# MMintLab/gelslim_depth

Hardware: AMD Instinct MI355X
Metric: train frames/sec (320x427) at batch 32 (higher is better)
Workload: dtype f32

## Files before the change

### gelslim_depth_amd/csrc/gsd_conv3x3_w2d.hip

```cpp
#include "gsd_conv3x3_host.h"

#include <cstdio>
#include <cstdlib>
#include <type_traits>

__device__ const float gsd_pad_w2d[2] = {0.f, __builtin_nanf("")};

typedef float f32x4v __attribute__((ext_vector_type(4), aligned(4)));
typedef float f32x2v __attribute__((ext_vector_type(2)));

struct W2DParams {
  SrcD src0, src1;
  DstD dst0, dst1;
  const float* wt;
  float* partials;
  const float* bw_raw;
  const float* bw_scale;
  const float* bw_shift;
  const float* bw_mean;
  const float* bw_invstd;
  int Cin, Cout, Mpad, nchunks, mblocks;
  int N, H, W;
  int TH, TW, TWq, tiles_y, tiles_x, WR, WC, WCp, PS, NPV;
  int NP, NI;
  int mgrp, pgrp, ptiles;
  int nslab;
  float* slabs;
};

namespace {
constexpr int W2D_BM = 64;
constexpr int W2D_WTILE = 96 * W2D_BM;
constexpr int NWP = 2;
}

template <class GetY>
__device__ __forceinline__ void w2d_epilogue(const W2DParams& P, const float* sBw, const int n, const int h0, const int w0, const int tr2,
                                             const int tq, const int vmask, const int m0, const int mh, const int ph, const int j,
                                             const int l16, const int pt, GetY get_y) {
  constexpr int BM = 64;
  int off0_0 = 0, off0_1 = 0, off1_0 = 0, off1_1 = 0, sm0_0 = 0, sm0_1 = 0, sm1_0 = 0, sm1_1 = 0;
#pragma unroll
  for (int a = 0; a < 2; ++a) {
    const int h = h0 + 2 * tr2 + a, w = w0 + 4 * tq;
    const int vm = (vmask >> (4 * a)) & 15;
    int hd = h - P.dst0.oh, wd = w - P.dst0.ow;
    if ((unsigned)hd < (unsigned)P.dst0.H) {
      (a == 0 ? off0_0 : off0_1) = hd * P.dst0.ws + wd;
#pragma unroll
      for (int i = 0; i < 4; ++i)
        if ((vm >> i & 1) && (unsigned)(wd + i) < (unsigned)P.dst0.W) (a == 0 ? sm0_0 : sm0_1) |= 1 << i;
    }
    hd = h - P.dst1.oh;
    wd = w - P.dst1.ow;
    if ((unsigned)hd < (unsigned)P.dst1.H) {
      (a == 0 ? off1_0 : off1_1) = hd * P.dst1.ws + wd;
#pragma unroll
      for (int i = 0; i < 4; ++i)
        if ((vm >> i & 1) && (unsigned)(wd + i) < (unsigned)P.dst1.W) (a == 0 ? sm1_0 : sm1_1) |= 1 << i;
    }
  }
  auto OFF0 = [&](int a) { return a == 0 ? off0_0 : off0_1; };
  auto OFF1 = [&](int a) { return a == 0 ? off1_0 : off1_1; };
  auto SM0 = [&](int a) { return a == 0 ? sm0_0 : sm0_1; };
  auto SM1 = [&](int a) { return a == 0 ? sm1_0 : sm1_1; };
  const long long lane0 = (long long)(j * 4) * P.dst0.cs, lane1 = (long long)(j * 4) * P.dst1.cs;
  float* const d0 = P.dst0.p + (long long)n * P.dst0.ns;
  float* const d1 = P.dst1.p + (long long)n * P.dst1.ns;
  float* const prow = P.partials != nullptr ? P.partials + (size_t)(pt * NWP + ph) * (2 * P.Mpad) : nullptr;

  if (P.bw_raw == nullptr) {
#pragma unroll
    for (int m = 0; m < 2; ++m) {
#pragma unroll
      for (int reg = 0; reg < 4; ++reg) {
        const int cu = m0 + mh * 32 + m * 16 + reg, co = cu + j * 4;
        const bool first = co < P.dst0.C;
        const int cd = first ? co : co - P.dst0.C;
        const bool co_ok = co < P.Cout && (first || cd < P.dst1.C);
        float* const plane = first ? d0 + (long long)cu * P.dst0.cs + lane0 : d1 + (long long)(cu - P.dst0.C) * P.dst1.cs + lane1;
        float y[2][4];
        get_y(m, reg, y);
        float s1 = 0.f, s2 = 0.f;
#pragma unroll
        for (int a = 0; a < 2; ++a) {
          const int sm = co_ok ? (first ? SM0(a) : SM1(a)) : 0;
          float* const px = plane + (first ? OFF0(a) : OFF1(a));
#pragma unroll
          for (int i = 0; i < 4; ++i) {
            if (sm >> i & 1) {
              s1 += y[a][i];
              s2 = fmaf(y[a][i], y[a][i], s2);
            }
          }
          if (sm == 15) {
            *reinterpret_cast<f32x4v*>(px) = f32x4{y[a][0], y[a][1], y[a][2], y[a][3]};
          } else {
#pragma unroll
            for (int i = 0; i < 4; ++i)
              if (sm >> i & 1) px[i] = y[a][i];
          }
        }
        if (prow != nullptr) {
          s1 = reduce16_to_lane15(s1);
          s2 = reduce16_to_lane15(s2);
          if (l16 == 15 && co < P.Mpad) {
            prow[co] = s1;
            prow[P.Mpad + co] = s2;
          }
        }
      }
    }
  } else {
#pragma unroll
    for (int m = 0; m < 2; ++m) {
#pragma unroll
      for (int reg = 0; reg < 4; ++reg) {
        const int cu = m0 + mh * 32 + m * 16 + reg, co = cu + j * 4;
        const long long cplane = (long long)n * P.dst0.ns + (co < P.Cout ? (long long)cu * P.dst0.cs + lane0 : 0);
        float xr[2][4];
#pragma unroll
        for (int a = 0; a < 2; ++a) {
          const float* const rp = P.bw_raw + cplane + OFF0(a);
          if (SM0(a) == 15) {
            const f32x4 t = *reinterpret_cast<const f32x4v*>(rp);
            xr[a][0] = t[0], xr[a][1] = t[1], xr[a][2] = t[2], xr[a][3] = t[3];
          } else {
#pragma unroll
            for (int i = 0; i < 4; ++i) xr[a][i] = (SM0(a) >> i & 1) ? rp[i] : 0.f;
          }
        }
        const int cl = mh * 32 + m * 16 + j * 4 + reg;
        const float bsc = sBw[cl], bsh = sBw[BM + cl], bmu = sBw[2 * BM + cl], bis = sBw[3 * BM + cl];
        float y[2][4];
        get_y(m, reg, y);
        float s1 = 0.f, s2 = 0.f;
#pragma unroll
        for (int a = 0; a < 2; ++a) {
          const int sm = co < P.Cout ? SM0(a) : 0;
          float* const px = d0 + ((long long)cu * P.dst0.cs + lane0) + OFF0(a);
#pragma unroll
          for (int i = 0; i < 4; ++i) {
            const float x = xr[a][i];
            const float dz = ((sm >> i & 1) && fmaf(x, bsc, bsh) > 0.f) ? y[a][i] : 0.f;
            y[a][i] = dz;
            s1 += dz;
            s2 = fmaf(dz, (x - bmu) * bis, s2);
          }
          if (sm == 15) {
            *reinterpret_cast<f32x4v*>(px) = f32x4{y[a][0], y[a][1], y[a][2], y[a][3]};
          } else {
#pragma unroll
            for (int i = 0; i < 4; ++i)
              if (sm >> i & 1) px[i] = y[a][i];
          }
        }
        if (prow != nullptr) {
          s1 = reduce16_to_lane15(s1);
          s2 = reduce16_to_lane15(s2);
          if (l16 == 15 && co < P.Mpad) {
            prow[co] = s1;
            prow[P.Mpad + co] = s2;
          }
        }
      }
    }
  }
}

template <bool PLAIN, int HM = 0, bool SPLIT = false>
__global__ __launch_bounds__(128 * NWP, 2) void conv3x3_w2d_kernel(const W2DParams P) {
  constexpr bool X4 = HM == 1, U4 = HM == 2, PC = HM != 0;
  constexpr int W2D_NONE = -2147483647 - 1, W2D_PAD = -2147483647;
  static_assert(!X4 || PLAIN, "aligned 16-byte halo pieces: a plain, row-pitched source");
  constexpr int BM = W2D_BM, WTILE = W2D_WTILE, NT = 128 * NWP, NW = 2 * NWP;
  extern __shared__ __attribute__((aligned(16))) float smem[];
  const int PS = P.PS;
  const int BUF = WTILE + 4 * PS;

  const int tid = threadIdx.x, lane = tid & 63;
  const int wave8 = __builtin_amdgcn_readfirstlane(tid >> 6);
  const int ph = wave8 % NWP, fh = wave8 / NWP;
  const int j = lane >> 4, l16 = lane & 15;

  const int lid = xcd_swizzle(blockIdx.x, gridDim.x);
  int mbb = lid % P.mblocks;
  const int slab = SPLIT ? (lid / P.mblocks) % P.nslab : 0;
  int pt = SPLIT ? lid / P.mblocks / P.nslab : lid / P.mblocks;
  if (!SPLIT && P.mgrp < P.mblocks) {
    const int gsz = P.pgrp * P.mblocks;
    const int g = lid / gsz;
    int r = lid - g * gsz;
    const int p0 = g * P.pgrp;
    const int pn = min(P.pgrp, P.ptiles - p0);
    const int per = pn * P.mgrp;
    const int mg = r / per;
    r -= mg * per;
    const int gn = min(P.mgrp, P.mblocks - mg * P.mgrp);
    const int pl = r / gn;
    pt = p0 + pl;
    mbb = mg * P.mgrp + (r - pl * gn);
  }
  const int c_lo = SPLIT ? (int)((long)slab * P.nchunks / P.nslab) : 0;
  const int c_hi = SPLIT ? (int)((long)(slab + 1) * P.nchunks / P.nslab) : P.nchunks;
  const int m0 = mbb * BM;
  const int tpi = P.tiles_y * P.tiles_x;
  const int n = pt / tpi;
  const int rt = pt - n * tpi;
  const int ty = rt / P.tiles_x;
  const int h0 = ty * P.TH, w0 = (rt - ty * P.tiles_x) * P.TW;

  const int q = ph * 16 + l16;
  const bool q_ok = q < (P.TH >> 1) * P.TWq && q < 16 * NWP;
  const int tr2 = q_ok ? q / P.TWq : 0;
  const int tq = q_ok ? q - tr2 * P.TWq : 0;
  const int baddr = WTILE + j * PS + (2 * tr2) * P.WCp + 4 * tq + (PC ? 4 : 0);
  int vmask = 0;
  if (q_ok) {
#pragma unroll
    for (int a = 0; a < 2; ++a)
      if (h0 + 2 * tr2 + a < P.H) {
#pragma unroll
        for (int i = 0; i < 4; ++i)
          if (w0 + 4 * tq + i < P.W) vmask |= 1 << (4 * a + i);
      }
  }

  bool p_on[2];
  int pmask = 0;
  auto seg_offsets = [&](const int seg, int (&xo)[2], const bool mark) __attribute__((always_inline)) {
    const SrcD& S = seg ? P.src1 : P.src0;
#pragma unroll
    for (int pp = 0; pp < 2; ++pp) {
      xo[pp] = W2D_NONE;
      if constexpr (PC) {
        const int u = wave8 + NW * pp;
        p_on[pp] = u < 4 * P.NI;
        const int piece = (u % P.NI) * 64 + lane;
        const int rr = piece / P.NP, pc = piece - rr * P.NP;
        if (rr < P.WR) {
          const int gh = h0 - 1 + rr, gw = w0 - 4 + 4 * pc;
          if constexpr (X4) {
            xo[pp] = ((unsigned)gh < (unsigned)S.H && gw >= 0 && gw + 4 <= S.ws) ? gh * S.ws + gw : W2D_PAD;
          } else {
            const int hs = gh - S.oh, c0 = gw - S.ow;
            xo[pp] = W2D_PAD;
            if (S.C > 0 && (unsigned)hs < (unsigned)S.H && c0 + 3 >= 0 && c0 < S.W) {
              xo[pp] = hs * S.ws + c0;
#pragma unroll
              for (int e = 0; e < 4; ++e)
                if (mark && (c0 + e < 0 || c0 + e >= S.W)) pmask |= 1 << (8 * seg + 4 * pp + e);
            }
          }
        }
        continue;
      }
      p_on[pp] = wave8 + NW * pp < P.NPV;
      const int pos = (wave8 + NW * pp) * 64 + lane;
      const int rr = pos / P.WCp, cc = pos - rr * P.WCp;
      if (rr < P.WR && cc < P.WC) {
        const int gh = h0 - 1 + rr, gw = w0 - 1 + cc;
        const int hs = gh - S.oh, ws = gw - S.ow;
        xo[pp] = ((unsigned)hs < (unsigned)S.H && (unsigned)ws < (unsigned)S.W) ? hs * S.ws + ws : W2D_PAD;
      }
    }
  };
  int xo0[2], xo1[2];
  seg_offsets(0, xo0, true);
  seg_offsets(1, xo1, true);
  const int f_sw = P.src1.C > 0 ? P.src0.C / 4 : -1;
  const bool start1 = SPLIT && f_sw >= 0 && c_lo >= f_sw;
  {
    const float pad0 = (start1 ? P.src1.relu : P.src0.relu) ? __builtin_nanf("") : 0.f;
#pragma unroll
    for (int pp = 0; pp < 2; ++pp)
      if (p_on[pp] && (start1 ? xo1[pp] : xo0[pp]) == W2D_PAD) {
#pragma unroll
        for (int b = 0; b < 2; ++b) {
          if constexpr (PC) {
            const int u = wave8 + NW * pp;
#pragma unroll
            for (int e = 0; e < 4; ++e) smem[b * BUF + WTILE + (u / P.NI) * PS + 1 + (u % P.NI) * 256 + lane * 4 + e] = pad0;
          } else {
#pragma unroll
            for (int ch = 0; ch < 4; ++ch) smem[b * BUF + WTILE + ch * PS + (wave8 + NW * pp) * 64 + lane] = pad0;
          }
        }
      }
  }
  long long d_cs = start1 ? P.src1.cs : P.src0.cs;
  const float* d_base = (start1 ? P.src1.p + (long long)n * P.src1.ns : P.src0.p + (long long)n * P.src0.ns) +
                        (long long)(c_lo - (start1 ? f_sw : 0)) * 4 * d_cs;
  long long f_xl[2];
#pragma unroll
  for (int pp = 0; pp < 2; ++pp) f_xl[pp] = start1 ? xo1[pp] : xo0[pp];
  auto begin_fill = [&](int chunk, int buf) {
    if (f_sw < 0 || start1 || (chunk != f_sw && chunk != f_sw + 1)) return;
    if (chunk == f_sw) {
      d_base = P.src1.p + (long long)n * P.src1.ns;
      d_cs = P.src1.cs;
      int xs[2];
      seg_offsets(1, xs, false);
#pragma unroll
      for (int pp = 0; pp < 2; ++pp) f_xl[pp] = xs[pp];
    }
    const float pad1 = P.src1.relu ? __builtin_nanf("") : 0.f;
#pragma unroll
    for (int pp = 0; pp < 2; ++pp)
      if (p_on[pp] && f_xl[pp] == W2D_PAD) {
        if constexpr (PC) {
          const int u = wave8 + NW * pp;
#pragma unroll
          for (int e = 0; e < 4; ++e) smem[buf * BUF + WTILE + (u / P.NI) * PS + 1 + (u % P.NI) * 256 + lane * 4 + e] = pad1;
        } else {
#pragma unroll
          for (int ch = 0; ch < 4; ++ch) smem[buf * BUF + WTILE + ch * PS + (wave8 + NW * pp) * 64 + lane] = pad1;
        }
      }
  };
  auto halo_slot = [&](int ch, float* Xb) {
#pragma unroll
    for (int pp = 0; pp < 2; ++pp)
      if (p_on[pp] && f_xl[pp] > W2D_PAD) __builtin_amdgcn_global_load_lds(d_base + f_xl[pp], Xb + ch * PS + (wave8 + NW * pp) * 64, 4, 0, 0);
    d_base += d_cs;
  };
  auto halo_unit = [&](int pp, float* Xb) {
    const int u = wave8 + NW * pp;
    if (p_on[pp] && f_xl[pp] > W2D_PAD)
      __builtin_amdgcn_global_load_lds(d_base + (u / P.NI) * d_cs + f_xl[pp], Xb + (u / P.NI) * PS + 1 + (u % P.NI) * 256, 16, 0, 0);
    if (pp == 1) d_base += 4 * d_cs;
  };
  constexpr int WPW = 24 / NW;
  const float* const wsrc0 = P.wt + (size_t)mbb * P.nchunks * WTILE + wave8 * (WPW * 256) + lane * 4;
  auto weight_fill = [&](int chunk, float* Wn) {
    const float* wg = wsrc0 + (size_t)chunk * WTILE;
    float* wl = Wn + wave8 * (WPW * 256);
    __builtin_amdgcn_global_load_lds(wg, wl, 16, 0, 0);
    __builtin_amdgcn_global_load_lds(wg, wl, 16, 1024, 0);
    __builtin_amdgcn_global_load_lds(wg, wl, 16, 2048, 0);
    if constexpr (WPW == 6) {
      __builtin_amdgcn_global_load_lds(wg, wl, 16, 3072, 0);
      __builtin_amdgcn_global_load_lds(wg + 1024, wl + 1024, 16, 0, 0);
      __builtin_amdgcn_global_load_lds(wg + 1024, wl + 1024, 16, 1024, 0);
    }
  };

  const int Kpad = P.nchunks * 4;
  float* sAff = smem + 2 * BUF;
  for (int c = tid; c < Kpad; c += NT) {
    const bool first = c < P.src0.C;
    const SrcD& S = first ? P.src0 : P.src1;
    const int cc = first ? c : c - P.src0.C;
    float sc = 1.f, sh = 0.f;
    if (c < P.Cin && cc < S.C && S.scale != nullptr) {
      sc = S.scale[cc];
      sh = S.shift[cc];
    }
    sAff[c] = sc;
    sAff[Kpad + c] = sh;
  }
  float* sBw = sAff + 2 * Kpad;
  if (P.bw_raw != nullptr) {
    for (int c = tid; c < BM; c += NT) {
      const int co = m0 + c < P.Cout ? m0 + c : 0;
      sBw[c] = P.bw_scale[co];
      sBw[BM + c] = P.bw_shift[co];
      sBw[2 * BM + c] = P.bw_mean[co];
      sBw[3 * BM + c] = P.bw_invstd[co];
    }
  }
  const float lo0 = P.src0.relu ? 0.f : -__builtin_inff(), lo1 = P.src1.relu ? 0.f : -__builtin_inff();

  const int rowA = baddr + (fh ? 2 : 0) * P.WCp, rowB = baddr + (fh ? 1 : 2) * P.WCp, rowC = baddr + (fh ? 3 : 1) * P.WCp;
  const f32x2v sg2 = {fh ? -1.f : 1.f, fh ? -1.f : 1.f};

  f32x4 acc[4][12];
#pragma unroll
  for (int m = 0; m < 4; ++m)
#pragma unroll
    for (int f = 0; f < 12; ++f) acc[m][f] = f32x4{0.f, 0.f, 0.f, 0.f};

  const int a_keep = (j * 12 + fh * 6) * 128 + l16 * 4 + fh * 64, a_give = a_keep + (fh ? -64 : 64);
  begin_fill(c_lo, 0);
  weight_fill(c_lo, smem);
  if constexpr (PC) {
    halo_unit(0, smem + WTILE);
    halo_unit(1, smem + WTILE);
  } else {
#pragma unroll
    for (int ch = 0; ch < 4; ++ch) halo_slot(ch, smem + WTILE);
  }

  auto run_chunk = [&](const int chunk, auto cur_c) {
    constexpr int cur = decltype(cur_c)::value;
    if constexpr (U4) {
      __builtin_amdgcn_s_waitcnt(0x0F70);
      const bool seg1 = f_sw >= 0 && chunk >= f_sw;
      const int pm = seg1 ? pmask >> 8 : pmask & 0xff;
      if (pm != 0) {
        const float padv = (seg1 ? P.src1.relu : P.src0.relu) ? __builtin_nanf("") : 0.f;
#pragma unroll
        for (int pp = 0; pp < 2; ++pp) {
          const int u = wave8 + NW * pp;
          float* pq = smem + cur * BUF + WTILE + (u / P.NI) * PS + 1 + (u % P.NI) * 256 + lane * 4;
#pragma unroll
          for (int e = 0; e < 4; ++e)
            if (pm >> (4 * pp + e) & 1) pq[e] = padv;
        }
      }
      __syncthreads();
    } else {
      gsd_dma_barrier();
    }
    const int kc = chunk * 4 + j;
    float sc = 1.f, sh = 0.f, lo = 0.f;
    if constexpr (!PLAIN) {
      sc = sAff[kc], sh = sAff[Kpad + kc];
      lo = kc < P.src0.C ? lo0 : (kc < P.Cin ? lo1 : -__builtin_inff());
    }
    const bool more = chunk + 1 < c_hi;
    int ioff = cur * BUF;
    __asm__ volatile("" : "+s"(ioff));
    const float* Wc = smem + ioff;
    auto load_row = [&](const int addr, float (&r)[6]) {
      const f32x4 ra = *reinterpret_cast<const f32x4*>(&Wc[addr]);
      const f32x2v rb = *reinterpret_cast<const f32x2v*>(&Wc[addr + 4]);
      r[0] = ra[0], r[1] = ra[1], r[2] = ra[2], r[3] = ra[3], r[4] = rb[0], r[5] = rb[1];
    };
    float dA[6], dB[6], dC[6];
    load_row(rowA, dA);
    load_row(rowB, dB);
    load_row(rowC, dC);
    f32x4 av[2];
    av[0] = *reinterpret_cast<const f32x4*>(&Wc[a_keep]);
    auto affine = [&](float (&r)[6]) {
      if constexpr (!PLAIN) {
        const f32x2v sc2 = {sc, sc}, sh2 = {sh, sh};
#pragma unroll
        for (int c = 0; c < 6; c += 2) {
          const f32x2v y = __builtin_elementwise_fma(f32x2v{r[c], r[c + 1]}, sc2, sh2);
          r[c] = fmaxf(y[0], lo);
          r[c + 1] = fmaxf(y[1], lo);
        }
      }
    };
    const f32x2v m41 = {-4.f, -1.f}, p1m1 = {1.f, -1.f}, p2m2 = {2.f, -2.f}, m5 = {-5.f, -5.f}, p4 = {4.f, 4.f};
    auto rt_a = [&](const f32x2v (&tp)[3], f32x2v& ac, f32x2v& be) {
      ac = __builtin_elementwise_fma(f32x2v{tp[1][0], tp[1][0]}, m41, f32x2v{tp[2][0], tp[2][0]});
      be = __builtin_elementwise_fma(f32x2v{tp[0][1], tp[0][1]}, m41, f32x2v{tp[1][1], tp[1][1]});
    };
    auto rt_b = [&](const f32x2v& ac, const f32x2v& be, float (&v)[6]) {
      const f32x2v v12 = __builtin_elementwise_fma(f32x2v{be[0], be[0]}, p1m1, f32x2v{ac[0], ac[0]});
      const f32x2v v34 = __builtin_elementwise_fma(f32x2v{be[1], be[1]}, p2m2, f32x2v{ac[1], ac[1]});
      v[1] = v12[0], v[2] = v12[1], v[3] = v34[0], v[4] = v34[1];
    };
    auto rt_c = [&](const f32x2v (&tp)[3], float (&v)[6]) {
      const f32x2v v05 = __builtin_elementwise_fma(tp[0], p4, __builtin_elementwise_fma(tp[1], m5, tp[2]));
      v[0] = v05[0], v[5] = v05[1];
    };
    affine(dA);
    affine(dB);
    f32x2v tA[3], tB[3], acB, beB;
#pragma unroll
    for (int k = 0; k < 3; ++k) tA[k] = f32x2v{dA[2 * k], dA[2 * k + 1]} - f32x2v{dB[2 * k], dB[2 * k + 1]};
    auto col_b = [&]() {
#pragma unroll
      for (int k = 0; k < 3; ++k)
        tB[k] = __builtin_elementwise_fma(f32x2v{dC[2 * k], dC[2 * k + 1]}, sg2, f32x2v{dB[2 * k], dB[2 * k + 1]});
    };
    if constexpr (!PLAIN) {
      affine(dC);
      col_b();
    }
    float v[2][6];
    {
      f32x2v ac, be;
      rt_a(tA, ac, be);
      rt_b(ac, be, v[0]);
      rt_c(tA, v[0]);
    }
    __builtin_amdgcn_sched_barrier(0);
#pragma unroll
    for (int g = 0; g < 12; ++g) {
      const int r = g / 6, fe = (g >> 1) * 2 - 6 * r, mt = 2 * (g & 1);
      if (g + 1 < 12) av[(g + 1) & 1] = *reinterpret_cast<const f32x4*>(&Wc[((g + 1) & 1 ? a_give : a_keep) + ((g + 1) >> 1) * 128]);
      const f32x4& ap = av[g & 1];
      acc[mt][6 * r + fe] = mfma16(ap[0], v[r][fe], acc[mt][6 * r + fe]);
      acc[mt + 1][6 * r + fe] = mfma16(ap[1], v[r][fe], acc[mt + 1][6 * r + fe]);
      acc[mt][6 * r + fe + 1] = mfma16(ap[2], v[r][fe + 1], acc[mt][6 * r + fe + 1]);
      acc[mt + 1][6 * r + fe + 1] = mfma16(ap[3], v[r][fe + 1], acc[mt + 1][6 * r + fe + 1]);
      const int piece = PLAIN ? g + 1 : g + 2;
      if (piece == 1) col_b();
      if (piece == 2) rt_a(tB, acB, beB);
      if (piece == 3) rt_b(acB, beB, v[1]);
      if (piece == 4) rt_c(tB, v[1]);
      if (more && g < 3) {
        float* Wn = smem + (cur ^ 1) * BUF;
        if (g == 0) {
          begin_fill(chunk + 1, cur ^ 1);
          weight_fill(chunk + 1, Wn);
        } else {
          if constexpr (PC) {
            halo_unit(g - 1, Wn + WTILE);
          } else {
            halo_slot(2 * g - 2, Wn + WTILE);
            halo_slot(2 * g - 1, Wn + WTILE);
          }
        }
      }
      if (g < 6) {
#pragma unroll
        for (int i = 0; i < 4; ++i) {
          __builtin_amdgcn_sched_group_barrier(0x008, 1, 0);
          __builtin_amdgcn_sched_group_barrier(0x002, 1, 0);
        }
      }
      __builtin_amdgcn_sched_barrier(0);
    }
  };
  for (int chunk = c_lo; chunk < c_hi; chunk += 2) {
    run_chunk(chunk, std::integral_constant<int, 0>{});
    if (chunk + 1 < c_hi) run_chunk(chunk + 1, std::integral_constant<int, 1>{});
  }

  {
    float* const xs = smem + (wave8 * 12) * 256 + lane * 4;
    const float* const xr = smem + ((ph + NWP * (1 - fh)) * 12) * 256 + lane * 4;
#pragma unroll
    for (int r = 0; r < 2; ++r) {
      __syncthreads();
#pragma unroll
      for (int f = 0; f < 12; ++f) *reinterpret_cast<f32x4*>(xs + f * 256) = acc[2 + r][f];
      __syncthreads();
#pragma unroll
      for (int f = 0; f < 12; ++f) acc[2 + r][f] = *reinterpret_cast<const f32x4*>(xr + f * 256);
    }
  }

  auto out_transform = [&](auto hi_c, int m, int reg, float (&y)[2][4]) __attribute__((always_inline)) {
    constexpr bool HI = decltype(hi_c)::value;
    const int lo = HI ? 2 + m : m, hi = HI ? m : 2 + m;
    const int r0 = reg & ~1;
#pragma unroll
    for (int a = 0; a < 2; ++a) {
      f32x2v R[6];
#pragma unroll
      for (int fc = 0; fc < 6; ++fc) {
        const f32x2v M0 = {acc[lo][fc][r0], acc[lo][fc][r0 + 1]}, M1 = {acc[lo][6 + fc][r0], acc[lo][6 + fc][r0 + 1]};
        const f32x2v M2 = {acc[hi][fc][r0], acc[hi][fc][r0 + 1]}, M3 = {acc[hi][6 + fc][r0], acc[hi][6 + fc][r0 + 1]};
        R[fc] = a == 0 ? M0 + M1 + M2 : M1 - M2 - M3;
      }
      const f32x2v p12 = R[1] + R[2], m12 = R[1] - R[2], p34 = R[3] + R[4], m34 = R[3] - R[4];
      const f32x2v c2 = {2.f, 2.f}, c4 = {4.f, 4.f}, c8 = {8.f, 8.f};
      const f32x2v y0 = R[0] + p12 + p34, y1 = __builtin_elementwise_fma(c2, m34, m12), y2 = __builtin_elementwise_fma(c4, p34, p12);
      const f32x2v y3 = __builtin_elementwise_fma(c8, m34, m12) + R[5];
      y[a][0] = y0[reg & 1], y[a][1] = y1[reg & 1], y[a][2] = y2[reg & 1], y[a][3] = y3[reg & 1];
    }
  };

  auto finish = [&](auto hi_c) __attribute__((always_inline)) {
    auto get_y = [&](int m, int reg, float (&y)[2][4]) __attribute__((always_inline)) { out_transform(hi_c, m, reg, y); };
    if constexpr (SPLIT) {
      float* const sl = P.slabs + ((size_t)((size_t)pt * P.nslab + slab) * P.mblocks + mbb) * (size_t)(BM * 128 * NWP);
#pragma unroll
      for (int m = 0; m < 2; ++m)
#pragma unroll
        for (int reg = 0; reg < 4; ++reg) {
          float y[2][4];
          get_y(m, reg, y);
          float* const o = sl + ((size_t)(fh * 32 + m * 16 + j * 4 + reg) * (16 * NWP) + q) * 8;
          *reinterpret_cast<f32x4*>(o) = f32x4{y[0][0], y[0][1], y[0][2], y[0][3]};
          *reinterpret_cast<f32x4*>(o + 4) = f32x4{y[1][0], y[1][1], y[1][2], y[1][3]};
        }
    } else {
      w2d_epilogue(P, sBw, n, h0, w0, tr2, tq, vmask, m0, fh, ph, j, l16, pt, get_y);
    }
  };
  if (fh == 0)
    finish(std::false_type{});
  else
    finish(std::true_type{});
}

__global__ __launch_bounds__(128 * NWP) void w2d_slab_reduce_kernel(const W2DParams P) {
  constexpr int BM = W2D_BM;
  __shared__ float sBw[4 * BM];
  const int tid = threadIdx.x, lane = tid & 63;
  const int wave8 = __builtin_amdgcn_readfirstlane(tid >> 6);
  const int ph = wave8 % NWP, mh = wave8 / NWP;
  const int j = lane >> 4, l16 = lane & 15;
  const int lid = xcd_swizzle(blockIdx.x, gridDim.x);
  const int mbb = lid % P.mblocks;
  const int pt = lid / P.mblocks;
  const int m0 = mbb * BM;
  const int tpi = P.tiles_y * P.tiles_x;
  const int n = pt / tpi;
  const int rt = pt - n * tpi;
  const int ty = rt / P.tiles_x;
  const int h0 = ty * P.TH, w0 = (rt - ty * P.tiles_x) * P.TW;
  const int q = ph * 16 + l16;
  const bool q_ok = q < (P.TH >> 1) * P.TWq && q < 16 * NWP;
  const int tr2 = q_ok ? q / P.TWq : 0;
  const int tq = q_ok ? q - tr2 * P.TWq : 0;
  int vmask = 0;
  if (q_ok) {
#pragma unroll
    for (int a = 0; a < 2; ++a)
      if (h0 + 2 * tr2 + a < P.H) {
#pragma unroll
        for (int i = 0; i < 4; ++i)
          if (w0 + 4 * tq + i < P.W) vmask |= 1 << (4 * a + i);
      }
  }
  if (P.bw_raw != nullptr) {
    for (int c = tid; c < BM; c += 128 * NWP) {
      const int co = m0 + c < P.Cout ? m0 + c : 0;
      sBw[c] = P.bw_scale[co];
      sBw[BM + c] = P.bw_shift[co];
      sBw[2 * BM + c] = P.bw_mean[co];
      sBw[3 * BM + c] = P.bw_invstd[co];
    }
    __syncthreads();
  }
  const size_t tile_elems = (size_t)(BM * 128 * NWP);
  const float* const s0 = P.slabs + ((size_t)pt * P.nslab * P.mblocks + mbb) * tile_elems;
  auto get_y = [&](int m, int reg, float (&y)[2][4]) __attribute__((always_inline)) {
    const float* o = s0 + ((size_t)(mh * 32 + m * 16 + j * 4 + reg) * (16 * NWP) + q) * 8;
    f32x4 a = *reinterpret_cast<const f32x4*>(o), b = *reinterpret_cast<const f32x4*>(o + 4);
    for (int s = 1; s < P.nslab; ++s) {
      o += (size_t)P.mblocks * tile_elems;
      a += *reinterpret_cast<const f32x4*>(o);
      b += *reinterpret_cast<const f32x4*>(o + 4);
    }
    y[0][0] = a[0], y[0][1] = a[1], y[0][2] = a[2], y[0][3] = a[3];
    y[1][0] = b[0], y[1][1] = b[1], y[1][2] = b[2], y[1][3] = b[3];
  };
  w2d_epilogue(P, sBw, n, h0, w0, tr2, tq, vmask, m0, mh, ph, j, l16, pt, get_y);
}

namespace {

struct W2DPlan {
  int TH, TW, TWq, tiles_y, tiles_x, mblocks, WR, WC, WCp, PS;
};

bool plan_w2d(int N, int H, int W, int M, W2DPlan* best) {
  long best_cost = -1;
  const int force_tw = gsd_env_int("GSD_W2D_TW", 0);
  const int maxpos = 256 * NWP;
  static const int tws[4] = {32, 64, 16, 8};
  for (int k = 0; k < 4; ++k) {
    const int tw = tws[k];
    if (force_tw && tw != force_tw) continue;
    const int twq = tw / 4;
    int th = 2 * (16 * NWP / twq);
    const int wcp0 = round_up(tw + 2, 4);
    if ((th + 2) * wcp0 > maxpos) continue;
    const int ty = ceil_div(H, th);
    th = round_up(ceil_div(H, ty), 2);
    const long blocks = (long)ty * ceil_div(W, tw) * N;
    const long cost = (blocks * 8 + (tw == 32 ? 0 : tw == 64 ? 1 : tw == 16 ? 2 : 3)) * (tw == 8 ? 100 + gsd_env_int("GSD_W2D_TW8_PCT", 8) : 100);
    if (best_cost < 0 || cost < best_cost) {
      best_cost = cost;
      best->TH = th; best->TW = tw; best->TWq = twq;
      best->tiles_y = ty; best->tiles_x = ceil_div(W, tw);
      best->WR = th + 2; best->WC = tw + 2;
    }
  }
  best->mblocks = ceil_div(M, W2D_BM);
  if (best_cost < 0) return false;
  static std::atomic<uint64_t> memo[16];
  const int th = best->TH, tw = best->TW, key = (th << 16) | (tw << 4);
  std::atomic<uint64_t>& mm = memo[(th * 7 + tw) & 15];
  {
    const uint64_t v = mm.load(std::memory_order_acquire);
    if (v != 0 && (int)(v >> 40) == key) {
      best->WCp = (int)(v >> 20) & 0xFFFFF;
      best->PS = (int)v & 0xFFFFF;
      return true;
    }
  }
  const int wcp0 = round_up(tw + 2, 4);
  int bc = -1;
  for (int c = wcp0; c <= wcp0 + 12 && (th + 2) * c <= maxpos; c += 4)
    for (int ps = round_up((th + 2) * c, 4) + 4; ps < round_up((th + 2) * c, 4) + 4 + 36; ps += 4) {
      const int cyc = conv3_halo_read_cycles(NWP, 2, best->TWq, c, ps, 0);
      if (bc < 0 || cyc < bc) {
        bc = cyc;
        best->WCp = c;
        best->PS = ps;
      }
    }
  if (key < (1 << 24) && best->WCp < (1 << 20) && best->PS < (1 << 20))
    mm.store(((uint64_t)key << 40) | ((uint64_t)best->WCp << 20) | (uint64_t)best->PS, std::memory_order_release);
  return true;
}

int w2d_x4_plane_stride(int TWq, int WCp, int WR) {
  static std::atomic<uint64_t> memo[8];
  const int key = (TWq << 20) | (WCp << 8) | WR;
  std::atomic<uint64_t>& mm = memo[(TWq + WR) & 7];
  {
    const uint64_t v = mm.load(std::memory_order_acquire);
    if (v != 0 && (int)(v >> 32) == key) return (int)(v & 0xFFFFFFFFu);
  }
  int best = -1, ps_best = WR * WCp + 4;
  for (int ps = WR * WCp + 4; ps < WR * WCp + 4 + 68; ps += 4) {
    const int c = conv3_halo_read_cycles(NWP, 2, TWq, WCp, ps, 0);
    if (best < 0 || c < best) {
      best = c;
      ps_best = ps;
    }
  }
  mm.store(((uint64_t)(unsigned)key << 32) | (uint64_t)(unsigned)ps_best, std::memory_order_release);
  return ps_best;
}

template <bool PLAIN, int HM = 0, bool SPLIT = false>
int launch_w2d(const W2DParams& P, int grid, size_t lds, hipStream_t st) {
  if (int e = gsd_launch<conv3x3_w2d_kernel<PLAIN, HM, SPLIT>>("gsd_conv3x3_w2d", dim3(grid), dim3(128 * NWP), lds, st, P)) return e;
  if constexpr (SPLIT) {
    hipLaunchKernelGGL(w2d_slab_reduce_kernel, dim3(grid / P.nslab), dim3(128 * NWP), 0, st, P);
    GSD_LAUNCH_CHECK("gsd_conv3x3_w2d (slab sums)");
  }
  return GSD_OK;
}

constexpr Conv3SlabModel w2d_slabs = {2.07, 5.0, 0.66, "GSD_W2D_SPLIT"};

}

extern "C" int gsd_conv3x3_w2d_supported(int Cin, int C0) {
  return (Cin > 0 && Cin % 4 == 0 && C0 > 0 && C0 <= Cin && C0 % 4 == 0) ? 1 : 0;
}

extern "C" int gsd_conv3x3_w2d_partial_rows(int N, int H, int W, int Cout) {
  if (N <= 0 || H <= 0 || W <= 0 || Cout <= 0) return 0;
  W2DPlan p;
  if (!plan_w2d(N, H, W, Cout, &p)) return 0;
  return N * p.tiles_y * p.tiles_x * NWP;
}

extern "C" int64_t gsd_conv3x3_w2d_mfma_count(int N, int H, int W, int Cin, int Cout) {
  W2DPlan p;
  if (N <= 0 || H <= 0 || W <= 0 || Cin <= 0 || Cout <= 0 || !plan_w2d(N, H, W, Cout, &p)) return 0;
  return (int64_t)N * p.tiles_y * p.tiles_x * p.mblocks * ceil_div(Cin, 4) * (2 * NWP * 48);
}

extern "C" double gsd_conv3x3_w2d_estimate_us(int N, int H, int W, int Cin, int Cout) {
  W2DPlan p;
  if (N <= 0 || H <= 0 || W <= 0 || Cin <= 0 || Cout <= 0 || !plan_w2d(N, H, W, Cout, &p)) return 0.0;
  const long blocks = (long)N * p.tiles_y * p.tiles_x * p.mblocks;
  return w2d_slabs.time_us(blocks, ceil_div(Cin, 4), 1, false);
}

extern "C" double gsd_conv3x3_w2d_estimate_slabs_us(int N, int H, int W, int Cin, int Cout) {
  W2DPlan p;
  if (N <= 0 || H <= 0 || W <= 0 || Cin <= 0 || Cout <= 0 || !plan_w2d(N, H, W, Cout, &p)) return 0.0;
  const long blocks = (long)N * p.tiles_y * p.tiles_x * p.mblocks;
  return w2d_slabs.time_us(blocks, ceil_div(Cin, 4), w2d_slabs.pick(blocks, ceil_div(Cin, 4), false), false);
}

extern "C" int64_t gsd_conv3x3_w2d_workspace(int N, int H, int W, int Cin, int Cout) {
  W2DPlan p;
  if (N <= 0 || H <= 0 || W <= 0 || Cin <= 0 || Cout <= 0 || Cin % 4 != 0 || !plan_w2d(N, H, W, Cout, &p)) return 0;
  const long blocks = (long)N * p.tiles_y * p.tiles_x * p.mblocks;
  const int S = std::max(w2d_slabs.pick(blocks, Cin / 4, false), w2d_slabs.pick(blocks, Cin / 4, true));
  return S > 1 ? (int64_t)blocks * S * (W2D_BM * 256) : 0;
}

extern "C" int gsd_conv3x3_prefers_w2d(int N, int H, int W, int Cin, int Cout, int train) {
  if (N <= 0 || H <= 0 || W <= 0 || Cin < 16 || Cin % 4 != 0 || Cout <= 0) return 0;
  const int forced = gsd_env_int("GSD_CONV_W2D", -1);
  if (forced == 0 || forced == 1) return forced;
  if (!train) return 1;
  const double a = gsd_conv3x3_w2d_estimate_slabs_us(N, H, W, Cin, Cout), b = gsd_conv3x3_w43_estimate_us(N, H, W, Cin, Cout, 1);
  return a > 0.0 && b > 0.0 && a < b ? 1 : 0;
}

static int w2d_impl(const gsd_src* src, int nsrc, const float* wt, int Cin, int Cout, const gsd_dst* dst, int ndst, float* partials,
                    const Conv3Bw& bw, int N, int H, int W, void* stream, float* ws = nullptr, int64_t ws_elems = 0) {
  if (int e = conv3_check_operands("gsd_conv3x3_w2d", true, true, src, nsrc, wt, Cin, Cout, dst, ndst, N, H, W)) return e;
  GSD_REQUIRE(gsd_conv3x3_w2d_supported(Cin, src[0].C), GSD_ERR_UNSUPPORTED,
              "gsd_conv3x3_w2d: Cin=%d and the first segment's %d channels must be multiples of 4 (use gsd_conv3x3_w43)", Cin, src[0].C);

  W2DPlan pl;
  GSD_REQUIRE(plan_w2d(N, H, W, Cout, &pl), GSD_ERR_UNSUPPORTED, "gsd_conv3x3_w2d: no tile shape");
  W2DParams P;
  conv3_fill_common(P, src, nsrc, wt, Cin, Cout, dst, ndst, partials, bw, N, H, W);
  P.mblocks = pl.mblocks;
  P.TH = pl.TH; P.TW = pl.TW; P.TWq = pl.TWq; P.tiles_y = pl.tiles_y; P.tiles_x = pl.tiles_x;
  P.WR = pl.WR; P.WC = pl.WC; P.WCp = pl.WCp; P.PS = pl.PS;
  P.NPV = ceil_div(P.WR * P.WCp, 64);
  GSD_REQUIRE(P.NPV <= 4 * NWP, GSD_ERR_UNSUPPORTED, "gsd_conv3x3_w2d: halo window too large");
  {
    int g = (gsd_env_int("GSD_W2D_L2KB", 3072) << 10) / (P.nchunks * W2D_WTILE * 4);
    const int forced = gsd_env_int("GSD_W2D_MGROUP", -1);
    if (forced == 0) g = P.mblocks;
    if (forced > 0) g = forced;
    P.mgrp = std::min(std::max(g, 1), P.mblocks);
    P.pgrp = std::max(gsd_env_int("GSD_W2D_PGROUP", 64 / P.mgrp), 1);
    P.ptiles = N * pl.tiles_y * pl.tiles_x;
  }
  const long base = (long)N * pl.tiles_y * pl.tiles_x * P.mblocks;
  int S = ws != nullptr ? w2d_slabs.pick(base, P.nchunks, bw.raw != nullptr) : 1;
  while (S > 1 && (int64_t)base * S * (W2D_BM * 256) > ws_elems) --S;
  if (S > 1 && P.nchunks / S < 2) S = 1;
  P.nslab = S;
  P.slabs = S > 1 ? ws : nullptr;
  if (S > 1) GSD_REQUIRE(((uintptr_t)ws & 15) == 0, GSD_ERR_BAD_ARG, "gsd_conv3x3_w2d: the K-slab workspace must be 16-byte aligned");
  const long grid = base * S;
  GSD_REQUIRE(grid < 2147483647L, GSD_ERR_UNSUPPORTED, "gsd_conv3x3_w2d: grid too large");
  bool plain = true;
  for (int i = 0; i < nsrc; ++i) plain = plain && src[i].scale == nullptr && src[i].relu == 0;
  P.NP = pl.TW / 4 + 2;
  P.NI = ceil_div(P.WR * P.NP, 64);
  const bool x4 = plain && nsrc == 1 && 4 * P.NI <= 8 && gsd_env_int("GSD_W2D_X4", 1) != 0 &&
                  ((uintptr_t)src[0].ptr & 15) == 0 && src[0].w_stride % 4 == 0 && src[0].c_stride % 4 == 0 && src[0].n_stride % 4 == 0 &&
                  src[0].off_h == 0 && src[0].off_w == 0 && src[0].w_stride >= round_up(src[0].W, 4);
  bool u4 = !x4 && 4 * P.NI <= 8 && gsd_env_int("GSD_W2D_U4", 1) != 0;
  for (int i = 0; i < nsrc && u4; ++i) u4 = src[i].slack >= 4;
  if (x4 || u4) {
    P.WCp = 4 * P.NP;
    P.PS = w2d_x4_plane_stride(pl.TWq, P.WCp, P.WR);
  }
  const size_t lds = (size_t)(2 * (W2D_WTILE + 4 * P.PS) + 2 * 4 * P.nchunks + 4 * W2D_BM) * sizeof(float);
  if (gsd_env_set("GSD_W2D_TRACE"))
    fprintf(stderr, "w2d M%d K%d %dx%d N%d nsrc %d ndst %d plain %d x4 %d u4 %d | ptr&15 %d ws %d cs%%4 %d ns%%4 %d NI %d tile %dx%d slabs %d\n", Cout, Cin, H, W, N,
            nsrc, ndst, (int)plain, (int)x4, (int)u4, (int)((uintptr_t)src[0].ptr & 15), src[0].w_stride, (int)(src[0].c_stride % 4),
            (int)(src[0].n_stride % 4), P.NI, pl.TH, pl.TW, S);
  if (S > 1) {
    if (x4) return launch_w2d<true, 1, true>(P, (int)grid, lds, (hipStream_t)stream);
    if (u4) return plain ? launch_w2d<true, 2, true>(P, (int)grid, lds, (hipStream_t)stream) : launch_w2d<false, 2, true>(P, (int)grid, lds, (hipStream_t)stream);
    return plain ? launch_w2d<true, 0, true>(P, (int)grid, lds, (hipStream_t)stream) : launch_w2d<false, 0, true>(P, (int)grid, lds, (hipStream_t)stream);
  }
  if (x4) return launch_w2d<true, 1>(P, (int)grid, lds, (hipStream_t)stream);
  if (u4) return plain ? launch_w2d<true, 2>(P, (int)grid, lds, (hipStream_t)stream) : launch_w2d<false, 2>(P, (int)grid, lds, (hipStream_t)stream);
  return plain ? launch_w2d<true>(P, (int)grid, lds, (hipStream_t)stream) : launch_w2d<false>(P, (int)grid, lds, (hipStream_t)stream);
}

extern "C" int gsd_conv3x3_w2d(const gsd_src* src, int nsrc, const float* wt, int Cin, int Cout, const gsd_dst* dst, int ndst,
                               float* partials, int N, int H, int W, void* stream) {
  return w2d_impl(src, nsrc, wt, Cin, Cout, dst, ndst, partials, Conv3Bw{}, N, H, W, stream);
}

extern "C" int gsd_conv3x3_w2d_dgrad_bnrelu(const gsd_src* src, const float* wt, int Cin, int Cout, const gsd_dst* dst,
                                            const float* raw, const float* scale, const float* shift, const float* mean,
                                            const float* invstd, float* partials, int N, int H, int W, void* stream) {
  return gsd_conv3x3_w2d_dgrad_bnrelu_ws(src, wt, Cin, Cout, dst, raw, scale, shift, mean, invstd, partials, nullptr, 0, N, H, W, stream);
}

extern "C" int gsd_conv3x3_w2d_ws(const gsd_src* src, int nsrc, const float* wt, int Cin, int Cout, const gsd_dst* dst, int ndst,
                                  float* partials, float* workspace, int64_t workspace_elems, int N, int H, int W, void* stream) {
  return w2d_impl(src, nsrc, wt, Cin, Cout, dst, ndst, partials, Conv3Bw{}, N, H, W, stream, workspace, workspace_elems);
}

extern "C" int gsd_conv3x3_w2d_dgrad_bnrelu_ws(const gsd_src* src, const float* wt, int Cin, int Cout, const gsd_dst* dst,
                                               const float* raw, const float* scale, const float* shift, const float* mean,
                                               const float* invstd, float* partials, float* workspace, int64_t workspace_elems, int N,
                                               int H, int W, void* stream) {
  const Conv3Bw bw{raw, scale, shift, mean, invstd};
  if (int e = conv3_check_dgrad_bnrelu("gsd_conv3x3_w2d_dgrad_bnrelu", dst, bw, partials, Cout, H, W)) return e;
  return w2d_impl(src, 1, wt, Cin, Cout, dst, 1, partials, bw, N, H, W, stream, workspace, workspace_elems);
}
```

Measured before the change: 369.5.

## Streamline w2d conv addressing: magic division, fast-path epilogue, paired outputs, scalar hints

```diff
diff --git a/gelslim_depth_amd/csrc/gsd_conv3x3_w2d.hip b/gelslim_depth_amd/csrc/gsd_conv3x3_w2d.hip
--- a/gelslim_depth_amd/csrc/gsd_conv3x3_w2d.hip
+++ b/gelslim_depth_amd/csrc/gsd_conv3x3_w2d.hip
@@ -8,6 +8,28 @@
 
 typedef float f32x4v __attribute__((ext_vector_type(4), aligned(4)));
 typedef float f32x2v __attribute__((ext_vector_type(2)));
+typedef __attribute__((address_space(1))) f32x4v g_f32x4v;
+typedef __attribute__((address_space(1))) float g_float;
+typedef __attribute__((address_space(1))) char g_char;
+__device__ __forceinline__ g_f32x4v* w2d_g4(g_char* base, unsigned off) { return (g_f32x4v*)(base + off); }
+__device__ __forceinline__ g_float* w2d_g1(g_char* base, unsigned off) { return (g_float*)(base + off); }
+
+struct W2DDiv {
+  unsigned mul, s1, s2;
+};
+static inline W2DDiv w2d_div_of(unsigned d) {
+  unsigned l = 0;
+  while ((1ull << l) < d) ++l;
+  W2DDiv r;
+  r.mul = (unsigned)(((1ull << 32) * ((1ull << l) - d)) / d + 1);
+  r.s1 = l < 1 ? l : 1;
+  r.s2 = l > 0 ? l - 1 : 0;
+  return r;
+}
+__device__ __forceinline__ int w2d_div(int x, const W2DDiv& d) {
+  const unsigned t = __umulhi((unsigned)x, d.mul);
+  return (int)((t + (((unsigned)x - t) >> d.s1)) >> d.s2);
+}
 
 struct W2DParams {
   SrcD src0, src1;
@@ -24,6 +46,9 @@
   int TH, TW, TWq, tiles_y, tiles_x, WR, WC, WCp, PS, NPV;
   int NP, NI;
   int mgrp, pgrp, ptiles;
+  W2DDiv d_mblocks, d_nslab, d_tpi, d_tiles_x, d_NP, d_WCp;
+  int TWq_sh;
+  int dfast;
   int nslab;
   float* slabs;
 };
@@ -34,11 +59,83 @@
 constexpr int NWP = 2;
 }
 
-template <class GetY>
+template <class GetPair>
 __device__ __forceinline__ void w2d_epilogue(const W2DParams& P, const float* sBw, const int n, const int h0, const int w0, const int tr2,
                                              const int tq, const int vmask, const int m0, const int mh, const int ph, const int j,
-                                             const int l16, const int pt, GetY get_y) {
+                                             const int l16, const int pt, GetPair get_pair) {
   constexpr int BM = 64;
+  float* const prow = P.partials != nullptr ? P.partials + (size_t)(pt * NWP + ph) * (2 * P.Mpad) : nullptr;
+  const int mc = m0 + mh * 32;
+  {
+    const bool in1 = mc >= P.dst0.C;
+    const int d_oh = in1 ? P.dst1.oh : P.dst0.oh, d_ow = in1 ? P.dst1.ow : P.dst0.ow, d_H = in1 ? P.dst1.H : P.dst0.H;
+    const int d_W = in1 ? P.dst1.W : P.dst0.W, d_ws = in1 ? P.dst1.ws : P.dst0.ws;
+    const long long d_cs = in1 ? P.dst1.cs : P.dst0.cs, d_ns = in1 ? P.dst1.ns : P.dst0.ns;
+    const int hd = h0 + 2 * tr2 - d_oh, wd = w0 + 4 * tq - d_ow;
+    const bool lane_in = vmask == 0xff && hd >= 0 && hd + 2 <= d_H && wd >= 0 && wd + 4 <= d_W;
+    const bool chan_in = (in1 ? mc + 32 <= P.Cout : mc + 32 <= P.dst0.C) && (P.dfast >> (in1 ? 1 : 0) & 1) != 0;
+    if (chan_in && __builtin_amdgcn_ballot_w64(lane_in) == ~0ull) {
+      unsigned o0 = ((unsigned)(j * 4) * (unsigned)d_cs + (unsigned)(hd * d_ws + wd)) * 4u;
+      unsigned o1 = o0 + (unsigned)d_ws * 4u;
+      unsigned oj = (unsigned)j * 16u;
+      asm volatile("" : "+v"(o0), "+v"(o1), "+v"(oj));
+      const long long pl0 = (long long)n * d_ns + (long long)(mc - (in1 ? P.dst0.C : 0)) * d_cs;
+#pragma unroll
+      for (int p = 0; p < 4; ++p) {
+      float y[2][2][4], s1v[2], s2v[2];
+      get_pair(p, y);
+#pragma unroll
+      for (int c = 0; c < 2; ++c) {
+        const int cw = (p >> 1) * 16 + (p & 1) * 2 + c;
+        g_char* dp = (g_char*)((in1 ? P.dst1.p : P.dst0.p) + pl0 + (long long)cw * d_cs);
+        asm volatile("" : "+s"(dp));
+        float s1 = 0.f, s2 = 0.f;
+        if (P.bw_raw == nullptr) {
+#pragma unroll
+          for (int a = 0; a < 2; ++a)
+#pragma unroll
+            for (int i = 0; i < 4; ++i) {
+              s1 += y[c][a][i];
+              s2 = fmaf(y[c][a][i], y[c][a][i], s2);
+            }
+        } else {
+          g_char* rp = (g_char*)(P.bw_raw + pl0 + (long long)cw * d_cs);
+          asm volatile("" : "+s"(rp));
+          asm volatile("" : "+v"(o0), "+v"(o1));
+          const f32x4 x0 = *w2d_g4(rp, o0), x1 = *w2d_g4(rp, o1);
+          const int cl = mh * 32 + (p >> 1) * 16 + j * 4 + (p & 1) * 2 + c;
+          const float bsc = sBw[cl], bsh = sBw[BM + cl], bmu = sBw[2 * BM + cl], bis = sBw[3 * BM + cl];
+#pragma unroll
+          for (int a = 0; a < 2; ++a)
+#pragma unroll
+            for (int i = 0; i < 4; ++i) {
+              const float x = a == 0 ? x0[i] : x1[i];
+              const float dz = fmaf(x, bsc, bsh) > 0.f ? y[c][a][i] : 0.f;
+              y[c][a][i] = dz;
+              s1 += dz;
+              s2 = fmaf(dz, (x - bmu) * bis, s2);
+            }
+        }
+        asm volatile("" : "+v"(o0), "+v"(o1));
+        *w2d_g4(dp, o0) = f32x4{y[c][0][0], y[c][0][1], y[c][0][2], y[c][0][3]};
+        *w2d_g4(dp, o1) = f32x4{y[c][1][0], y[c][1][1], y[c][1][2], y[c][1][3]};
+        s1v[c] = reduce16_to_lane15(s1);
+        s2v[c] = reduce16_to_lane15(s2);
+      }
+      if (prow != nullptr && l16 == 15) {
+#pragma unroll
+        for (int c = 0; c < 2; ++c) {
+          g_char* pp = (g_char*)(prow + mc + (p >> 1) * 16 + (p & 1) * 2 + c);
+          asm volatile("" : "+s"(pp));
+          asm volatile("" : "+v"(oj));
+          *w2d_g1(pp, oj) = s1v[c];
+          *w2d_g1(pp + (size_t)P.Mpad * 4, oj) = s2v[c];
+        }
+      }
+      }
+      return;
+    }
+  }
   int off0_0 = 0, off0_1 = 0, off1_0 = 0, off1_1 = 0, sm0_0 = 0, sm0_1 = 0, sm1_0 = 0, sm1_1 = 0;
 #pragma unroll
   for (int a = 0; a < 2; ++a) {
@@ -67,104 +164,86 @@
   const long long lane0 = (long long)(j * 4) * P.dst0.cs, lane1 = (long long)(j * 4) * P.dst1.cs;
   float* const d0 = P.dst0.p + (long long)n * P.dst0.ns;
   float* const d1 = P.dst1.p + (long long)n * P.dst1.ns;
-  float* const prow = P.partials != nullptr ? P.partials + (size_t)(pt * NWP + ph) * (2 * P.Mpad) : nullptr;
-
-  if (P.bw_raw == nullptr) {
-#pragma unroll
-    for (int m = 0; m < 2; ++m) {
-#pragma unroll
-      for (int reg = 0; reg < 4; ++reg) {
-        const int cu = m0 + mh * 32 + m * 16 + reg, co = cu + j * 4;
-        const bool first = co < P.dst0.C;
-        const int cd = first ? co : co - P.dst0.C;
-        const bool co_ok = co < P.Cout && (first || cd < P.dst1.C);
-        float* const plane = first ? d0 + (long long)cu * P.dst0.cs + lane0 : d1 + (long long)(cu - P.dst0.C) * P.dst1.cs + lane1;
-        float y[2][4];
-        get_y(m, reg, y);
-        float s1 = 0.f, s2 = 0.f;
-#pragma unroll
-        for (int a = 0; a < 2; ++a) {
-          const int sm = co_ok ? (first ? SM0(a) : SM1(a)) : 0;
-          float* const px = plane + (first ? OFF0(a) : OFF1(a));
-#pragma unroll
-          for (int i = 0; i < 4; ++i) {
-            if (sm >> i & 1) {
-              s1 += y[a][i];
-              s2 = fmaf(y[a][i], y[a][i], s2);
-            }
+
+#pragma unroll
+  for (int p = 0; p < 4; ++p) {
+  float y[2][2][4];
+  get_pair(p, y);
+#pragma unroll
+  for (int c = 0; c < 2; ++c) {
+    const int m = p >> 1, reg = (p & 1) * 2 + c;
+    const int cu = mc + m * 16 + reg, co = cu + j * 4;
+    float s1 = 0.f, s2 = 0.f;
+    if (P.bw_raw == nullptr) {
+      const bool first = co < P.dst0.C;
+      const int cd = first ? co : co - P.dst0.C;
+      const bool co_ok = co < P.Cout && (first || cd < P.dst1.C);
+      float* const plane = first ? d0 + (long long)cu * P.dst0.cs + lane0 : d1 + (long long)(cu - P.dst0.C) * P.dst1.cs + lane1;
+#pragma unroll
+      for (int a = 0; a < 2; ++a) {
+        const int sm = co_ok ? (first ? SM0(a) : SM1(a)) : 0;
+        float* const px = plane + (first ? OFF0(a) : OFF1(a));
+#pragma unroll
+        for (int i = 0; i < 4; ++i) {
+          if (sm >> i & 1) {
+            s1 += y[c][a][i];
+            s2 = fmaf(y[c][a][i], y[c][a][i], s2);
           }
-          if (sm == 15) {
-            *reinterpret_cast<f32x4v*>(px) = f32x4{y[a][0], y[a][1], y[a][2], y[a][3]};
-          } else {
-#pragma unroll
-            for (int i = 0; i < 4; ++i)
-              if (sm >> i & 1) px[i] = y[a][i];
-          }
-        }
-        if (prow != nullptr) {
-          s1 = reduce16_to_lane15(s1);
-          s2 = reduce16_to_lane15(s2);
-          if (l16 == 15 && co < P.Mpad) {
-            prow[co] = s1;
-            prow[P.Mpad + co] = s2;
-          }
-        }
-      }
-    }
-  } else {
-#pragma unroll
-    for (int m = 0; m < 2; ++m) {
-#pragma unroll
-      for (int reg = 0; reg < 4; ++reg) {
-        const int cu = m0 + mh * 32 + m * 16 + reg, co = cu + j * 4;
-        const long long cplane = (long long)n * P.dst0.ns + (co < P.Cout ? (long long)cu * P.dst0.cs + lane0 : 0);
-        float xr[2][4];
-#pragma unroll
-        for (int a = 0; a < 2; ++a) {
-          const float* const rp = P.bw_raw + cplane + OFF0(a);
-          if (SM0(a) == 15) {
-            const f32x4 t = *reinterpret_cast<const f32x4v*>(rp);
-            xr[a][0] = t[0], xr[a][1] = t[1], xr[a][2] = t[2], xr[a][3] = t[3];
-          } else {
-#pragma unroll
-            for (int i = 0; i < 4; ++i) xr[a][i] = (SM0(a) >> i & 1) ? rp[i] : 0.f;
-          }
-        }
-        const int cl = mh * 32 + m * 16 + j * 4 + reg;
-        const float bsc = sBw[cl], bsh = sBw[BM + cl], bmu = sBw[2 * BM + cl], bis = sBw[3 * BM + cl];
-        float y[2][4];
-        get_y(m, reg, y);
-        float s1 = 0.f, s2 = 0.f;
-#pragma unroll
-        for (int a = 0; a < 2; ++a) {
-          const int sm = co < P.Cout ? SM0(a) : 0;
-          float* const px = d0 + ((long long)cu * P.dst0.cs + lane0) + OFF0(a);
-#pragma unroll
-          for (int i = 0; i < 4; ++i) {
-            const float x = xr[a][i];
-            const float dz = ((sm >> i & 1) && fmaf(x, bsc, bsh) > 0.f) ? y[a][i] : 0.f;
-            y[a][i] = dz;
-            s1 += dz;
-            s2 = fmaf(dz, (x - bmu) * bis, s2);
-          }
-          if (sm == 15) {
-            *reinterpret_cast<f32x4v*>(px) = f32x4{y[a][0], y[a][1], y[a][2], y[a][3]};
-          } else {
-#pragma unroll
-            for (int i = 0; i < 4; ++i)
-              if (sm >> i & 1) px[i] = y[a][i];
-          }
-        }
-        if (prow != nullptr) {
-          s1 = reduce16_to_lane15(s1);
-          s2 = reduce16_to_lane15(s2);
-          if (l16 == 15 && co < P.Mpad) {
-            prow[co] = s1;
-            prow[P.Mpad + co] = s2;
-          }
-        }
-      }
-    }
+        }
+        if (sm == 15) {
+          *reinterpret_cast<f32x4v*>(px) = f32x4{y[c][a][0], y[c][a][1], y[c][a][2], y[c][a][3]};
+        } else {
+#pragma unroll
+          for (int i = 0; i < 4; ++i)
+            if (sm >> i & 1) px[i] = y[c][a][i];
+        }
+      }
+    } else {
+      const long long cplane = (long long)n * P.dst0.ns + (co < P.Cout ? (long long)cu * P.dst0.cs + lane0 : 0);
+      float xr[2][4];
+#pragma unroll
+      for (int a = 0; a < 2; ++a) {
+        const float* const rp = P.bw_raw + cplane + OFF0(a);
+        if (SM0(a) == 15) {
+          const f32x4 t = *reinterpret_cast<const f32x4v*>(rp);
+          xr[a][0] = t[0], xr[a][1] = t[1], xr[a][2] = t[2], xr[a][3] = t[3];
+        } else {
+#pragma unroll
+          for (int i = 0; i < 4; ++i) xr[a][i] = (SM0(a) >> i & 1) ? rp[i] : 0.f;
+        }
+      }
+      const int cl = mh * 32 + m * 16 + j * 4 + reg;
+      const float bsc = sBw[cl], bsh = sBw[BM + cl], bmu = sBw[2 * BM + cl], bis = sBw[3 * BM + cl];
+#pragma unroll
+      for (int a = 0; a < 2; ++a) {
+        const int sm = co < P.Cout ? SM0(a) : 0;
+        float* const px = d0 + ((long long)cu * P.dst0.cs + lane0) + OFF0(a);
+#pragma unroll
+        for (int i = 0; i < 4; ++i) {
+          const float x = xr[a][i];
+          const float dz = ((sm >> i & 1) && fmaf(x, bsc, bsh) > 0.f) ? y[c][a][i] : 0.f;
+          y[c][a][i] = dz;
+          s1 += dz;
+          s2 = fmaf(dz, (x - bmu) * bis, s2);
+        }
+        if (sm == 15) {
+          *reinterpret_cast<f32x4v*>(px) = f32x4{y[c][a][0], y[c][a][1], y[c][a][2], y[c][a][3]};
+        } else {
+#pragma unroll
+          for (int i = 0; i < 4; ++i)
+            if (sm >> i & 1) px[i] = y[c][a][i];
+        }
+      }
+    }
+    if (prow != nullptr) {
+      s1 = reduce16_to_lane15(s1);
+      s2 = reduce16_to_lane15(s2);
+      if (l16 == 15 && co < P.Mpad) {
+        prow[co] = s1;
+        prow[P.Mpad + co] = s2;
+      }
+    }
+  }
   }
 }
 
@@ -172,11 +251,13 @@
 __global__ __launch_bounds__(128 * NWP, 2) void conv3x3_w2d_kernel(const W2DParams P) {
   constexpr bool X4 = HM == 1, U4 = HM == 2, PC = HM != 0;
   constexpr int W2D_NONE = -2147483647 - 1, W2D_PAD = -2147483647;
+  constexpr unsigned W2D_OFF_PAD = 0xFFFFFFFFu;
   static_assert(!X4 || PLAIN, "aligned 16-byte halo pieces: a plain, row-pitched source");
   constexpr int BM = W2D_BM, WTILE = W2D_WTILE, NT = 128 * NWP, NW = 2 * NWP;
   extern __shared__ __attribute__((aligned(16))) float smem[];
   const int PS = P.PS;
   const int BUF = WTILE + 4 * PS;
+  const int Kpad = P.nchunks * 4;
 
   const int tid = threadIdx.x, lane = tid & 63;
   const int wave8 = __builtin_amdgcn_readfirstlane(tid >> 6);
@@ -184,9 +265,10 @@
   const int j = lane >> 4, l16 = lane & 15;
 
   const int lid = xcd_swizzle(blockIdx.x, gridDim.x);
-  int mbb = lid % P.mblocks;
-  const int slab = SPLIT ? (lid / P.mblocks) % P.nslab : 0;
-  int pt = SPLIT ? lid / P.mblocks / P.nslab : lid / P.mblocks;
+  const int lid_m = w2d_div(lid, P.d_mblocks);
+  int mbb = lid - lid_m * P.mblocks;
+  int pt = SPLIT ? w2d_div(lid_m, P.d_nslab) : lid_m;
+  const int slab = SPLIT ? lid_m - pt * P.nslab : 0;
   if (!SPLIT && P.mgrp < P.mblocks) {
     const int gsz = P.pgrp * P.mblocks;
     const int g = lid / gsz;
@@ -201,18 +283,18 @@
     pt = p0 + pl;
     mbb = mg * P.mgrp + (r - pl * gn);
   }
-  const int c_lo = SPLIT ? (int)((long)slab * P.nchunks / P.nslab) : 0;
-  const int c_hi = SPLIT ? (int)((long)(slab + 1) * P.nchunks / P.nslab) : P.nchunks;
+  const int c_lo = SPLIT ? __builtin_amdgcn_readfirstlane((int)((long)slab * P.nchunks / P.nslab)) : 0;
+  const int c_hi = SPLIT ? __builtin_amdgcn_readfirstlane((int)((long)(slab + 1) * P.nchunks / P.nslab)) : P.nchunks;
   const int m0 = mbb * BM;
   const int tpi = P.tiles_y * P.tiles_x;
-  const int n = pt / tpi;
+  const int n = w2d_div(pt, P.d_tpi);
   const int rt = pt - n * tpi;
-  const int ty = rt / P.tiles_x;
+  const int ty = w2d_div(rt, P.d_tiles_x);
   const int h0 = ty * P.TH, w0 = (rt - ty * P.tiles_x) * P.TW;
 
   const int q = ph * 16 + l16;
   const bool q_ok = q < (P.TH >> 1) * P.TWq && q < 16 * NWP;
-  const int tr2 = q_ok ? q / P.TWq : 0;
+  const int tr2 = q_ok ? q >> P.TWq_sh : 0;
   const int tq = q_ok ? q - tr2 * P.TWq : 0;
   const int baddr = WTILE + j * PS + (2 * tr2) * P.WCp + 4 * tq + (PC ? 4 : 0);
   int vmask = 0;
@@ -226,9 +308,12 @@
       }
   }
 
+  int geo = tr2 | tq << 8 | vmask << 16;
+  asm volatile("" : "+v"(geo));
+
   bool p_on[2];
   int pmask = 0;
-  auto seg_offsets = [&](const int seg, int (&xo)[2], const bool mark) __attribute__((always_inline)) {
+  auto seg_offsets = [&](const int seg, int (&xo)[2]) __attribute__((always_inline)) {
     const SrcD& S = seg ? P.src1 : P.src0;
 #pragma unroll
     for (int pp = 0; pp < 2; ++pp) {
@@ -236,8 +321,8 @@
       if constexpr (PC) {
         const int u = wave8 + NW * pp;
         p_on[pp] = u < 4 * P.NI;
-        const int piece = (u % P.NI) * 64 + lane;
-        const int rr = piece / P.NP, pc = piece - rr * P.NP;
+        const int piece = (u & (P.NI - 1)) * 64 + lane;
+        const int rr = w2d_div(piece, P.d_NP), pc = piece - rr * P.NP;
         if (rr < P.WR) {
           const int gh = h0 - 1 + rr, gw = w0 - 4 + 4 * pc;
           if constexpr (X4) {
@@ -249,7 +334,7 @@
               xo[pp] = hs * S.ws + c0;
 #pragma unroll
               for (int e = 0; e < 4; ++e)
-                if (mark && (c0 + e < 0 || c0 + e >= S.W)) pmask |= 1 << (8 * seg + 4 * pp + e);
+                if (c0 + e < 0 || c0 + e >= S.W) pmask |= 1 << (8 * seg + 4 * pp + e);
             }
           }
         }
@@ -257,7 +342,7 @@
       }
       p_on[pp] = wave8 + NW * pp < P.NPV;
       const int pos = (wave8 + NW * pp) * 64 + lane;
-      const int rr = pos / P.WCp, cc = pos - rr * P.WCp;
+      const int rr = w2d_div(pos, P.d_WCp), cc = pos - rr * P.WCp;
       if (rr < P.WR && cc < P.WC) {
         const int gh = h0 - 1 + rr, gw = w0 - 1 + cc;
         const int hs = gh - S.oh, ws = gw - S.ow;
@@ -265,11 +350,23 @@
       }
     }
   };
+  const int nis = P.NI >> 1;
+  int u_pl[2], u_lds[2];
+#pragma unroll
+  for (int pp = 0; pp < 2; ++pp) {
+    const int u = wave8 + NW * pp;
+    u_pl[pp] = u >> nis;
+    u_lds[pp] = (u >> nis) * PS + 1 + (u & (P.NI - 1)) * 256;
+  }
   int xo0[2], xo1[2];
-  seg_offsets(0, xo0, true);
-  seg_offsets(1, xo1, true);
+  seg_offsets(0, xo0);
+  seg_offsets(1, xo1);
   const int f_sw = P.src1.C > 0 ? P.src0.C / 4 : -1;
+  const int c_sw = f_sw >= 0 ? f_sw : 2147483647;
   const bool start1 = SPLIT && f_sw >= 0 && c_lo >= f_sw;
+  int pm_any0 = U4 ? __builtin_popcountll(__builtin_amdgcn_ballot_w64((pmask & 0xff) != 0)) : 0;
+  int pm_any1 = U4 ? __builtin_popcountll(__builtin_amdgcn_ballot_w64((pmask >> 8) != 0)) : 0;
+  asm volatile("" : "+s"(pm_any0), "+s"(pm_any1));
   {
     const float pad0 = (start1 ? P.src1.relu : P.src0.relu) ? __builtin_nanf("") : 0.f;
 #pragma unroll
@@ -278,9 +375,8 @@
 #pragma unroll
         for (int b = 0; b < 2; ++b) {
           if constexpr (PC) {
-            const int u = wave8 + NW * pp;
-#pragma unroll
-            for (int e = 0; e < 4; ++e) smem[b * BUF + WTILE + (u / P.NI) * PS + 1 + (u % P.NI) * 256 + lane * 4 + e] = pad0;
+#pragma unroll
+            for (int e = 0; e < 4; ++e) smem[b * BUF + WTILE + u_lds[pp] + lane * 4 + e] = pad0;
           } else {
 #pragma unroll
             for (int ch = 0; ch < 4; ++ch) smem[b * BUF + WTILE + ch * PS + (wave8 + NW * pp) * 64 + lane] = pad0;
@@ -288,30 +384,45 @@
         }
       }
   }
-  long long d_cs = start1 ? P.src1.cs : P.src0.cs;
-  const float* d_base = (start1 ? P.src1.p + (long long)n * P.src1.ns : P.src0.p + (long long)n * P.src0.ns) +
-                        (long long)(c_lo - (start1 ? f_sw : 0)) * 4 * d_cs;
-  long long f_xl[2];
-#pragma unroll
-  for (int pp = 0; pp < 2; ++pp) f_xl[pp] = start1 ? xo1[pp] : xo0[pp];
+  long long d_csb = (start1 ? P.src1.cs : P.src0.cs) * 4;
+  const char* d_base = reinterpret_cast<const char*>((start1 ? P.src1.p + (long long)n * P.src1.ns : P.src0.p + (long long)n * P.src0.ns) +
+                                                     (long long)(c_lo - (start1 ? f_sw : 0)) * 4 * (d_csb >> 2)) - 16;
+  unsigned f_off[2];
+  unsigned long long f_msk[2];
+  auto off_of = [&](const int xo) { return xo == W2D_PAD ? W2D_OFF_PAD : (xo > W2D_PAD ? (unsigned)(xo + 4) * 4u : 0u); };
+  auto lane_state = [&](const unsigned (&o)[2]) __attribute__((always_inline)) {
+#pragma unroll
+    for (int pp = 0; pp < 2; ++pp) {
+      f_off[pp] = o[pp];
+      f_msk[pp] = __builtin_amdgcn_ballot_w64(p_on[pp] && o[pp] + 1u > 1u);
+      asm volatile("" : "+s"(f_msk[pp]));
+    }
+  };
+  unsigned* const sSw = reinterpret_cast<unsigned*>(smem + 2 * BUF + 2 * Kpad + 4 * BM);
+  {
+    const unsigned o0[2] = {off_of(xo0[0]), off_of(xo0[1])}, o1[2] = {off_of(xo1[0]), off_of(xo1[1])};
+    if constexpr (!X4) sSw[tid] = o1[0], sSw[NT + tid] = o1[1];
+    if constexpr (U4) sSw[2 * NT + tid] = (unsigned)pmask;
+    lane_state(start1 ? o1 : o0);
+  }
   auto begin_fill = [&](int chunk, int buf) {
+    if constexpr (X4) return;
     if (f_sw < 0 || start1 || (chunk != f_sw && chunk != f_sw + 1)) return;
     if (chunk == f_sw) {
-      d_base = P.src1.p + (long long)n * P.src1.ns;
-      d_cs = P.src1.cs;
-      int xs[2];
-      seg_offsets(1, xs, false);
-#pragma unroll
-      for (int pp = 0; pp < 2; ++pp) f_xl[pp] = xs[pp];
+      d_base = reinterpret_cast<const char*>(P.src1.p + (long long)n * P.src1.ns) - 16;
+      d_csb = P.src1.cs * 4;
+      int t = tid;
+      asm volatile("" : "+v"(t));
+      const unsigned o1[2] = {sSw[t], sSw[NT + t]};
+      lane_state(o1);
     }
     const float pad1 = P.src1.relu ? __builtin_nanf("") : 0.f;
 #pragma unroll
     for (int pp = 0; pp < 2; ++pp)
-      if (p_on[pp] && f_xl[pp] == W2D_PAD) {
+      if (p_on[pp] && f_off[pp] == W2D_OFF_PAD) {
         if constexpr (PC) {
-          const int u = wave8 + NW * pp;
-#pragma unroll
-          for (int e = 0; e < 4; ++e) smem[buf * BUF + WTILE + (u / P.NI) * PS + 1 + (u % P.NI) * 256 + lane * 4 + e] = pad1;
+#pragma unroll
+          for (int e = 0; e < 4; ++e) smem[buf * BUF + WTILE + u_lds[pp] + lane * 4 + e] = pad1;
         } else {
 #pragma unroll
           for (int ch = 0; ch < 4; ++ch) smem[buf * BUF + WTILE + ch * PS + (wave8 + NW * pp) * 64 + lane] = pad1;
@@ -319,33 +430,47 @@
       }
   };
   auto halo_slot = [&](int ch, float* Xb) {
+    const char* b = d_base;
+    asm volatile("" : "+s"(b));
 #pragma unroll
     for (int pp = 0; pp < 2; ++pp)
-      if (p_on[pp] && f_xl[pp] > W2D_PAD) __builtin_amdgcn_global_load_lds(d_base + f_xl[pp], Xb + ch * PS + (wave8 + NW * pp) * 64, 4, 0, 0);
-    d_base += d_cs;
+      if (__builtin_amdgcn_inverse_ballot_w64(f_msk[pp])) {
+        asm volatile("" : "+v"(f_off[pp]));
+        __builtin_amdgcn_global_load_lds(reinterpret_cast<const float*>(b + f_off[pp]), Xb + ch * PS + (wave8 + NW * pp) * 64, 4, 0, 0);
+      }
+    d_base += d_csb;
   };
   auto halo_unit = [&](int pp, float* Xb) {
-    const int u = wave8 + NW * pp;
-    if (p_on[pp] && f_xl[pp] > W2D_PAD)
-      __builtin_amdgcn_global_load_lds(d_base + (u / P.NI) * d_cs + f_xl[pp], Xb + (u / P.NI) * PS + 1 + (u % P.NI) * 256, 16, 0, 0);
-    if (pp == 1) d_base += 4 * d_cs;
+    const char* b = d_base + u_pl[pp] * d_csb;
+    asm volatile("" : "+s"(b));
+    if (__builtin_amdgcn_inverse_ballot_w64(f_msk[pp])) {
+      asm volatile("" : "+v"(f_off[pp]));
+      __builtin_amdgcn_global_load_lds(reinterpret_cast<const float*>(b + f_off[pp]), Xb + u_lds[pp], 16, 0, 0);
+    }
+    if (pp == 1) d_base += 4 * d_csb;
   };
   constexpr int WPW = 24 / NW;
-  const float* const wsrc0 = P.wt + (size_t)mbb * P.nchunks * WTILE + wave8 * (WPW * 256) + lane * 4;
+  const char* const wsrc0 = reinterpret_cast<const char*>(P.wt + (size_t)mbb * P.nchunks * WTILE + wave8 * (WPW * 256));
+  unsigned w_off = (unsigned)lane * 16u;
   auto weight_fill = [&](int chunk, float* Wn) {
-    const float* wg = wsrc0 + (size_t)chunk * WTILE;
+    const char* wb = wsrc0 + (size_t)chunk * (WTILE * 4);
+    asm volatile("" : "+s"(wb));
+    asm volatile("" : "+v"(w_off));
+    const float* wg = reinterpret_cast<const float*>(wb + w_off);
     float* wl = Wn + wave8 * (WPW * 256);
     __builtin_amdgcn_global_load_lds(wg, wl, 16, 0, 0);
     __builtin_amdgcn_global_load_lds(wg, wl, 16, 1024, 0);
     __builtin_amdgcn_global_load_lds(wg, wl, 16, 2048, 0);
     if constexpr (WPW == 6) {
       __builtin_amdgcn_global_load_lds(wg, wl, 16, 3072, 0);
-      __builtin_amdgcn_global_load_lds(wg + 1024, wl + 1024, 16, 0, 0);
-      __builtin_amdgcn_global_load_lds(wg + 1024, wl + 1024, 16, 1024, 0);
+      const char* wb2 = wb + 4096;
+      asm volatile("" : "+s"(wb2));
+      const float* wg2 = reinterpret_cast<const float*>(wb2 + w_off);
+      __builtin_amdgcn_global_load_lds(wg2, wl + 1024, 16, 0, 0);
+      __builtin_amdgcn_global_load_lds(wg2, wl + 1024, 16, 1024, 0);
     }
   };
 
-  const int Kpad = P.nchunks * 4;
   float* sAff = smem + 2 * BUF;
   for (int c = tid; c < Kpad; c += NT) {
     const bool first = c < P.src0.C;
@@ -371,7 +496,7 @@
   }
   const float lo0 = P.src0.relu ? 0.f : -__builtin_inff(), lo1 = P.src1.relu ? 0.f : -__builtin_inff();
 
-  const int rowA = baddr + (fh ? 2 : 0) * P.WCp, rowB = baddr + (fh ? 1 : 2) * P.WCp, rowC = baddr + (fh ? 3 : 1) * P.WCp;
+  const int rowA = (2 * fh) * P.WCp, rowB = (2 - fh) * P.WCp, rowC = (1 + 2 * fh) * P.WCp;
   const f32x2v sg2 = {fh ? -1.f : 1.f, fh ? -1.f : 1.f};
 
   f32x4 acc[4][12];
@@ -380,7 +505,7 @@
 #pragma unroll
     for (int f = 0; f < 12; ++f) acc[m][f] = f32x4{0.f, 0.f, 0.f, 0.f};
 
-  const int a_keep = (j * 12 + fh * 6) * 128 + l16 * 4 + fh * 64, a_give = a_keep + (fh ? -64 : 64);
+  const int a_keep = (j * 12 + fh * 6) * 128 + l16 * 4 + fh * 64, a_give = 64 - 128 * fh;
   begin_fill(c_lo, 0);
   weight_fill(c_lo, smem);
   if constexpr (PC) {
@@ -395,14 +520,16 @@
     constexpr int cur = decltype(cur_c)::value;
     if constexpr (U4) {
       __builtin_amdgcn_s_waitcnt(0x0F70);
-      const bool seg1 = f_sw >= 0 && chunk >= f_sw;
-      const int pm = seg1 ? pmask >> 8 : pmask & 0xff;
-      if (pm != 0) {
+      const bool seg1 = chunk >= c_sw;
+      if ((seg1 ? pm_any1 : pm_any0) != 0) {
+        int t = tid;
+        asm volatile("" : "+v"(t));
+        const int pmk = (int)sSw[2 * NT + t];
+        const int pm = seg1 ? pmk >> 8 : pmk & 0xff;
         const float padv = (seg1 ? P.src1.relu : P.src0.relu) ? __builtin_nanf("") : 0.f;
 #pragma unroll
         for (int pp = 0; pp < 2; ++pp) {
-          const int u = wave8 + NW * pp;
-          float* pq = smem + cur * BUF + WTILE + (u / P.NI) * PS + 1 + (u % P.NI) * 256 + lane * 4;
+          float* pq = smem + cur * BUF + WTILE + u_lds[pp] + lane * 4;
 #pragma unroll
           for (int e = 0; e < 4; ++e)
             if (pm >> (4 * pp + e) & 1) pq[e] = padv;
@@ -416,21 +543,24 @@
     float sc = 1.f, sh = 0.f, lo = 0.f;
     if constexpr (!PLAIN) {
       sc = sAff[kc], sh = sAff[Kpad + kc];
-      lo = kc < P.src0.C ? lo0 : (kc < P.Cin ? lo1 : -__builtin_inff());
-    }
-    const bool more = chunk + 1 < c_hi;
-    int ioff = cur * BUF;
-    __asm__ volatile("" : "+s"(ioff));
+      lo = chunk < c_sw ? lo0 : lo1;
+    }
+    int more = (chunk + 1 - c_hi) >> 31;
+    more = __builtin_amdgcn_readfirstlane(more);
+    int ioff = cur * BUF, ioA = cur * BUF + rowA, ioB = cur * BUF + rowB, ioC = cur * BUF + rowC, ioG = cur * BUF + a_give;
+    __asm__ volatile("" : "+s"(ioff), "+s"(ioA), "+s"(ioB), "+s"(ioC), "+s"(ioG));
     const float* Wc = smem + ioff;
-    auto load_row = [&](const int addr, float (&r)[6]) {
-      const f32x4 ra = *reinterpret_cast<const f32x4*>(&Wc[addr]);
-      const f32x2v rb = *reinterpret_cast<const f32x2v*>(&Wc[addr + 4]);
+    const float* Wg = smem + ioG;
+    auto load_row = [&](const int io, float (&r)[6]) {
+      const float* Wr = smem + io;
+      const f32x4 ra = *reinterpret_cast<const f32x4*>(&Wr[baddr]);
+      const f32x2v rb = *reinterpret_cast<const f32x2v*>(&Wr[baddr + 4]);
       r[0] = ra[0], r[1] = ra[1], r[2] = ra[2], r[3] = ra[3], r[4] = rb[0], r[5] = rb[1];
     };
     float dA[6], dB[6], dC[6];
-    load_row(rowA, dA);
-    load_row(rowB, dB);
-    load_row(rowC, dC);
+    load_row(ioA, dA);
+    load_row(ioB, dB);
+    load_row(ioC, dC);
     f32x4 av[2];
     av[0] = *reinterpret_cast<const f32x4*>(&Wc[a_keep]);
     auto affine = [&](float (&r)[6]) {
@@ -483,7 +613,7 @@
 #pragma unroll
     for (int g = 0; g < 12; ++g) {
       const int r = g / 6, fe = (g >> 1) * 2 - 6 * r, mt = 2 * (g & 1);
-      if (g + 1 < 12) av[(g + 1) & 1] = *reinterpret_cast<const f32x4*>(&Wc[((g + 1) & 1 ? a_give : a_keep) + ((g + 1) >> 1) * 128]);
+      if (g + 1 < 12) av[(g + 1) & 1] = *reinterpret_cast<const f32x4*>(&((g + 1) & 1 ? Wg : Wc)[a_keep + ((g + 1) >> 1) * 128]);
       const f32x4& ap = av[g & 1];
       acc[mt][6 * r + fe] = mfma16(ap[0], v[r][fe], acc[mt][6 * r + fe]);
       acc[mt + 1][6 * r + fe] = mfma16(ap[1], v[r][fe], acc[mt + 1][6 * r + fe]);
@@ -494,7 +624,9 @@
       if (piece == 2) rt_a(tB, acB, beB);
       if (piece == 3) rt_b(acB, beB, v[1]);
       if (piece == 4) rt_c(tB, v[1]);
-      if (more && g < 3) {
+      int more_g = more;
+      asm volatile("" : "+s"(more_g));
+      if (g < 3 && more_g != 0) {
         float* Wn = smem + (cur ^ 1) * BUF;
         if (g == 0) {
           begin_fill(chunk + 1, cur ^ 1);
@@ -537,10 +669,13 @@
     }
   }
 
-  auto out_transform = [&](auto hi_c, int m, int reg, float (&y)[2][4]) __attribute__((always_inline)) {
+  int tid_e = tid;
+  asm volatile("" : "+v"(tid_e));
+  const int j_e = (tid_e & 63) >> 4, l16_e = tid_e & 15, q_e = ph * 16 + l16_e;
+  auto out_pair = [&](auto hi_c, const int p, float (&y)[2][2][4]) __attribute__((always_inline)) {
     constexpr bool HI = decltype(hi_c)::value;
+    const int m = p >> 1, r0 = (p & 1) * 2;
     const int lo = HI ? 2 + m : m, hi = HI ? m : 2 + m;
-    const int r0 = reg & ~1;
 #pragma unroll
     for (int a = 0; a < 2; ++a) {
       f32x2v R[6];
@@ -554,32 +689,33 @@
       const f32x2v c2 = {2.f, 2.f}, c4 = {4.f, 4.f}, c8 = {8.f, 8.f};
       const f32x2v y0 = R[0] + p12 + p34, y1 = __builtin_elementwise_fma(c2, m34, m12), y2 = __builtin_elementwise_fma(c4, p34, p12);
       const f32x2v y3 = __builtin_elementwise_fma(c8, m34, m12) + R[5];
-      y[a][0] = y0[reg & 1], y[a][1] = y1[reg & 1], y[a][2] = y2[reg & 1], y[a][3] = y3[reg & 1];
+#pragma unroll
+      for (int e = 0; e < 2; ++e) y[e][a][0] = y0[e], y[e][a][1] = y1[e], y[e][a][2] = y2[e], y[e][a][3] = y3[e];
     }
   };
-
-  auto finish = [&](auto hi_c) __attribute__((always_inline)) {
-    auto get_y = [&](int m, int reg, float (&y)[2][4]) __attribute__((always_inline)) { out_transform(hi_c, m, reg, y); };
-    if constexpr (SPLIT) {
-      float* const sl = P.slabs + ((size_t)((size_t)pt * P.nslab + slab) * P.mblocks + mbb) * (size_t)(BM * 128 * NWP);
-#pragma unroll
-      for (int m = 0; m < 2; ++m)
-#pragma unroll
-        for (int reg = 0; reg < 4; ++reg) {
-          float y[2][4];
-          get_y(m, reg, y);
-          float* const o = sl + ((size_t)(fh * 32 + m * 16 + j * 4 + reg) * (16 * NWP) + q) * 8;
-          *reinterpret_cast<f32x4*>(o) = f32x4{y[0][0], y[0][1], y[0][2], y[0][3]};
-          *reinterpret_cast<f32x4*>(o + 4) = f32x4{y[1][0], y[1][1], y[1][2], y[1][3]};
-        }
-    } else {
-      w2d_epilogue(P, sBw, n, h0, w0, tr2, tq, vmask, m0, fh, ph, j, l16, pt, get_y);
-    }
+  auto get_pair = [&](const int p, float (&y)[2][2][4]) __attribute__((always_inline)) {
+    if (fh == 0)
+      out_pair(std::false_type{}, p, y);
+    else
+      out_pair(std::true_type{}, p, y);
   };
-  if (fh == 0)
-    finish(std::false_type{});
-  else
-    finish(std::true_type{});
+
+  if constexpr (SPLIT) {
+    float* const sl = P.slabs + ((size_t)((size_t)pt * P.nslab + slab) * P.mblocks + mbb) * (size_t)(BM * 128 * NWP);
+#pragma unroll
+    for (int p = 0; p < 4; ++p) {
+      float y[2][2][4];
+      get_pair(p, y);
+#pragma unroll
+      for (int e = 0; e < 2; ++e) {
+        float* const o = sl + ((size_t)(fh * 32 + (p >> 1) * 16 + j_e * 4 + (p & 1) * 2 + e) * (16 * NWP) + q_e) * 8;
+        *reinterpret_cast<f32x4*>(o) = f32x4{y[e][0][0], y[e][0][1], y[e][0][2], y[e][0][3]};
+        *reinterpret_cast<f32x4*>(o + 4) = f32x4{y[e][1][0], y[e][1][1], y[e][1][2], y[e][1][3]};
+      }
+    }
+  } else {
+    w2d_epilogue(P, sBw, n, h0, w0, geo & 255, geo >> 8 & 255, geo >> 16 & 255, m0, fh, ph, j_e, l16_e, pt, get_pair);
+  }
 }
 
 __global__ __launch_bounds__(128 * NWP) void w2d_slab_reduce_kernel(const W2DParams P) {
@@ -590,17 +726,17 @@
   const int ph = wave8 % NWP, mh = wave8 / NWP;
   const int j = lane >> 4, l16 = lane & 15;
   const int lid = xcd_swizzle(blockIdx.x, gridDim.x);
-  const int mbb = lid % P.mblocks;
-  const int pt = lid / P.mblocks;
+  const int pt = w2d_div(lid, P.d_mblocks);
+  const int mbb = lid - pt * P.mblocks;
   const int m0 = mbb * BM;
   const int tpi = P.tiles_y * P.tiles_x;
-  const int n = pt / tpi;
+  const int n = w2d_div(pt, P.d_tpi);
   const int rt = pt - n * tpi;
-  const int ty = rt / P.tiles_x;
+  const int ty = w2d_div(rt, P.d_tiles_x);
   const int h0 = ty * P.TH, w0 = (rt - ty * P.tiles_x) * P.TW;
   const int q = ph * 16 + l16;
   const bool q_ok = q < (P.TH >> 1) * P.TWq && q < 16 * NWP;
-  const int tr2 = q_ok ? q / P.TWq : 0;
+  const int tr2 = q_ok ? q >> P.TWq_sh : 0;
   const int tq = q_ok ? q - tr2 * P.TWq : 0;
   int vmask = 0;
   if (q_ok) {
@@ -624,18 +760,21 @@
   }
   const size_t tile_elems = (size_t)(BM * 128 * NWP);
   const float* const s0 = P.slabs + ((size_t)pt * P.nslab * P.mblocks + mbb) * tile_elems;
-  auto get_y = [&](int m, int reg, float (&y)[2][4]) __attribute__((always_inline)) {
-    const float* o = s0 + ((size_t)(mh * 32 + m * 16 + j * 4 + reg) * (16 * NWP) + q) * 8;
-    f32x4 a = *reinterpret_cast<const f32x4*>(o), b = *reinterpret_cast<const f32x4*>(o + 4);
-    for (int s = 1; s < P.nslab; ++s) {
-      o += (size_t)P.mblocks * tile_elems;
-      a += *reinterpret_cast<const f32x4*>(o);
-      b += *reinterpret_cast<const f32x4*>(o + 4);
-    }
-    y[0][0] = a[0], y[0][1] = a[1], y[0][2] = a[2], y[0][3] = a[3];
-    y[1][0] = b[0], y[1][1] = b[1], y[1][2] = b[2], y[1][3] = b[3];
+  auto get_pair = [&](const int p, float (&y)[2][2][4]) __attribute__((always_inline)) {
+#pragma unroll
+    for (int e = 0; e < 2; ++e) {
+      const float* o = s0 + ((size_t)(mh * 32 + (p >> 1) * 16 + j * 4 + (p & 1) * 2 + e) * (16 * NWP) + q) * 8;
+      f32x4 a = *reinterpret_cast<const f32x4*>(o), b = *reinterpret_cast<const f32x4*>(o + 4);
+      for (int s = 1; s < P.nslab; ++s) {
+        o += (size_t)P.mblocks * tile_elems;
+        a += *reinterpret_cast<const f32x4*>(o);
+        b += *reinterpret_cast<const f32x4*>(o + 4);
+      }
+      y[e][0][0] = a[0], y[e][0][1] = a[1], y[e][0][2] = a[2], y[e][0][3] = a[3];
+      y[e][1][0] = b[0], y[e][1][1] = b[1], y[e][1][2] = b[2], y[e][1][3] = b[3];
+    }
   };
-  w2d_epilogue(P, sBw, n, h0, w0, tr2, tq, vmask, m0, mh, ph, j, l16, pt, get_y);
+  w2d_epilogue(P, sBw, n, h0, w0, tr2, tq, vmask, m0, mh, ph, j, l16, pt, get_pair);
 }
 
 namespace {
@@ -784,6 +923,9 @@
   GSD_REQUIRE(gsd_conv3x3_w2d_supported(Cin, src[0].C), GSD_ERR_UNSUPPORTED,
               "gsd_conv3x3_w2d: Cin=%d and the first segment's %d channels must be multiples of 4 (use gsd_conv3x3_w43)", Cin, src[0].C);
 
+  for (int i = 0; i < nsrc; ++i)
+    GSD_REQUIRE((int64_t)src[i].H * src[i].w_stride + 4 < (1LL << 30), GSD_ERR_UNSUPPORTED,
+                "gsd_conv3x3_w2d: a source plane must stay below 2^30 floats");
   W2DPlan pl;
   GSD_REQUIRE(plan_w2d(N, H, W, Cout, &pl), GSD_ERR_UNSUPPORTED, "gsd_conv3x3_w2d: no tile shape");
   W2DParams P;
@@ -810,6 +952,14 @@
   P.slabs = S > 1 ? ws : nullptr;
   if (S > 1) GSD_REQUIRE(((uintptr_t)ws & 15) == 0, GSD_ERR_BAD_ARG, "gsd_conv3x3_w2d: the K-slab workspace must be 16-byte aligned");
   const long grid = base * S;
+  P.d_mblocks = w2d_div_of(P.mblocks);
+  P.d_nslab = w2d_div_of(S);
+  P.d_tpi = w2d_div_of(pl.tiles_y * pl.tiles_x);
+  P.d_tiles_x = w2d_div_of(pl.tiles_x);
+  P.TWq_sh = pl.TWq == 2 ? 1 : pl.TWq == 4 ? 2 : pl.TWq == 8 ? 3 : 4;
+  P.dfast = 0;
+  for (int i = 0; i < ndst; ++i)
+    if (4 * (12 * (int64_t)dst[i].c_stride + (int64_t)dst[i].H * dst[i].w_stride) < (1LL << 32)) P.dfast |= 1 << i;
   GSD_REQUIRE(grid < 2147483647L, GSD_ERR_UNSUPPORTED, "gsd_conv3x3_w2d: grid too large");
   bool plain = true;
   for (int i = 0; i < nsrc; ++i) plain = plain && src[i].scale == nullptr && src[i].relu == 0;
@@ -824,7 +974,9 @@
     P.WCp = 4 * P.NP;
     P.PS = w2d_x4_plane_stride(pl.TWq, P.WCp, P.WR);
   }
-  const size_t lds = (size_t)(2 * (W2D_WTILE + 4 * P.PS) + 2 * 4 * P.nchunks + 4 * W2D_BM) * sizeof(float);
+  P.d_NP = w2d_div_of(P.NP);
+  P.d_WCp = w2d_div_of(P.WCp);
+  const size_t lds = (size_t)(2 * (W2D_WTILE + 4 * P.PS) + 2 * 4 * P.nchunks + 4 * W2D_BM + 3 * 128 * NWP) * sizeof(float);
   if (gsd_env_set("GSD_W2D_TRACE"))
     fprintf(stderr, "w2d M%d K%d %dx%d N%d nsrc %d ndst %d plain %d x4 %d u4 %d | ptr&15 %d ws %d cs%%4 %d ns%%4 %d NI %d tile %dx%d slabs %d\n", Cout, Cin, H, W, N,
             nsrc, ndst, (int)plain, (int)x4, (int)u4, (int)((uintptr_t)src[0].ptr & 15), src[0].w_stride, (int)(src[0].c_stride % 4),
```

New measurement: 376.6 (median of 6 runs). 1.02x the previous value.
